# yh-jun/SNR-Aligned_diffSE

Measured on AMD Instinct MI355X. Metric: utterances/sec (4 s @16 kHz, N=30 PC steps) at 1/2/4/8 MI355X; PESQ delta vs ref, higher is better.
Workload: dtype fp16; 1 GPU; C2: B=32 4 s/16 kHz clips per GPU, N=30 PC steps (reverse_diffusion + ald, 60 NFE/utt), OUVE SDE, NCSN++ nf=128, fp16; global_batch=32, per_gpu_batch=32, seq_len=512, parallelism=dp1 (utterance sharding)

## Files before the change

### snr-aligned_diffse_amd/csrc/conv.hip

```cpp
#include "conv_common.h"

#include <algorithm>
#include <type_traits>

using namespace snrse_conv;

namespace {

template <int NWM, int BN>
SNRSE_DEV void block_stats_flush(const ConvParams& p, const float* red, int blk_b, int blk_n0) {
  asm volatile("s_waitcnt lgkmcnt(0)" ::: "memory");
  __builtin_amdgcn_s_barrier();
  const int slot = blockIdx.x & (SNRSE_STAT_SLOTS - 1);
  for (int t = threadIdx.x; t < 2 * BN; t += blockDim.x) {
    float a = 0.f;
#pragma unroll
    for (int w = 0; w < NWM; ++w) a += red[w * 2 * BN + t];
    if (blk_n0 + (t >> 1) < p.Cout)
      unsafeAtomicAdd(&p.stats[stat_idx(blk_b, slot, blk_n0 + (t >> 1), p.Cout) + (t & 1)], (double)a);
  }
}

template <typename TO, int NWM, int BN, bool DEFER = false, int LA = 8>
SNRSE_DEV void epilogue_lds(const ConvParams& p, const f32x4 (&acc)[4][4], int mb, int nb, int lane, float* stage,
// ... 21 lines not shown
    bias[k] = (p.bias && nok) ? p.bias[n + k] : 0.f;
    cb[k] = 0.f;
    cw[k][0] = cw[k][1] = cw[k][2] = cw[k][3] = 0.f;
    if (p.comb_src && nok) {
      cw[k][0] = p.comb_w[(n + k) * 4 + 0]; cw[k][1] = p.comb_w[(n + k) * 4 + 1];
      cw[k][2] = p.comb_w[(n + k) * 4 + 2]; cw[k][3] = p.comb_w[(n + k) * 4 + 3];
      cb[k] = p.comb_b[n + k];
    }
  }
  const int m_last = min(mb + nvalid - 1, p.M - 1);
  const bool one_b = mb < p.M && (mb / HW) == (m_last / HW);
  const int slot = blockIdx.x & (SNRSE_STAT_SLOTS - 1);
  const bool seg = p.stats && !one_b && HW % RPP == 0;
  int seg_b = -1;
  if (p.temb && one_b && nok) {
    const float* tb = p.temb + (size_t)(mb / HW) * p.temb_stride + n;
#pragma unroll
    for (int k = 0; k < EPC; ++k) bias[k] += tb[k];
  }
  constexpr int NPASS = 64 / RPP;
  static_assert(LA >= 1 && LA <= NPASS, "lookahead");
  u32x4 rpre[NPASS];
  f32x4 qpre[NPASS];
  auto epi_issue = [&](int pass) {
    const int row = r0 + pass * RPP;
    const int m = mb + row;
    if (m < p.M && nok && row < nvalid) {
      if (p.res) rpre[pass] = *(const u32x4*)((const TO*)p.res + (size_t)m * p.res_ld + n);
      if (p.comb_src) qpre[pass] = *(const f32x4*)(p.comb_src + (size_t)m * 4);
    }
  };
#pragma unroll
  for (int pass = 0; pass < LA; ++pass) epi_issue(pass);
  float s1[EPC], s2[EPC];
#pragma unroll
  for (int k = 0; k < EPC; ++k) { s1[k] = 0.f; s2[k] = 0.f; }
  auto seg_flush = [&]() {
#pragma unroll
    for (int k = 0; k < EPC; ++k) {
#pragma unroll
      for (int o = NCH; o < 64; o <<= 1) {
        s1[k] += __shfl_xor(s1[k], o, 64);
        s2[k] += __shfl_xor(s2[k], o, 64);
      }
    }
    if (r0 == 0 && nok && seg_b >= 0 && (long long)seg_b * HW < p.M) {
      const size_t base = stat_idx(seg_b, slot, n, p.Cout);
#pragma unroll
      for (int k = 0; k < EPC; ++k) {
        unsafeAtomicAdd(&p.stats[base + 2 * k], (double)s1[k]);
        unsafeAtomicAdd(&p.stats[base + 2 * k + 1], (double)s2[k]);
      }
    }
#pragma unroll
    for (int k = 0; k < EPC; ++k) { s1[k] = 0.f; s2[k] = 0.f; }
  };
#pragma unroll
  for (int pass = 0; pass < NPASS; ++pass) {
    if (pass + LA < NPASS) epi_issue(pass + LA);
    const int row = r0 + pass * RPP;
    const int m = mb + row;
    if (seg) {
      const int bp = (mb + pass * RPP) / HW;
      if (bp != seg_b) {
        if (seg_b >= 0) seg_flush();
        seg_b = bp;
      }
    }
    if (m >= p.M || !nok || row >= nvalid) continue;
    float v[EPC];
    const float* sr = stage + row * LDR + cc * EPC;
#pragma unroll
    for (int k = 0; k < EPC; ++k) v[k] = sr[k] + bias[k];
    if (p.temb && !one_b) {
      const float* tb = p.temb + (size_t)(m / HW) * p.temb_stride + n;
#pragma unroll
      for (int k = 0; k < EPC; ++k) v[k] += tb[k];
    }
    if (p.res) epi_residual<TO>(rpre[pass], v);
#pragma unroll
    for (int k = 0; k < EPC; ++k) v[k] *= p.out_scale;
    if (p.comb_src) {
      const f32x4 q = qpre[pass];
#pragma unroll
      for (int k = 0; k < EPC; ++k) v[k] += q[0] * cw[k][0] + q[1] * cw[k][1] + q[2] * cw[k][2] + q[3] * cw[k][3] + cb[k];
    }
    const u32x4 o = epi_pack<TO>(v);
    if (p.epi_nt)
      __builtin_nontemporal_store(o, (u32x4*)((TO*)p.out + (size_t)m * p.out_ld + n));
    else
      *(u32x4*)((TO*)p.out + (size_t)m * p.out_ld + n) = o;
    if (p.stats) {
      if (one_b || seg) {
#pragma unroll
        for (int k = 0; k < EPC; ++k) { s1[k] += v[k]; s2[k] = fmaf(v[k], v[k], s2[k]); }
      } else {
#pragma unroll
        for (int k = 0; k < EPC; ++k) {
          const size_t o = stat_idx(m / HW, slot, n + k, p.Cout);
          unsafeAtomicAdd(&p.stats[o], (double)v[k]);
          unsafeAtomicAdd(&p.stats[o + 1], (double)v[k] * v[k]);
        }
      }
    }
  }
  if (seg && seg_b >= 0) seg_flush();
  if (p.stats && one_b) {
#pragma unroll
    for (int k = 0; k < EPC; ++k) {
#pragma unroll
      for (int o = NCH; o < 64; o <<= 1) {
        s1[k] += __shfl_xor(s1[k], o, 64);
        s2[k] += __shfl_xor(s2[k], o, 64);
      }
    }
  }
  if (p.stats && blk_b >= 0) {
    if (r0 == 0) {
#pragma unroll
      for (int k = 0; k < EPC; ++k) {
        red[(wm * BN + nb - blk_n0 + cc * EPC + k) * 2] = s1[k];
        red[(wm * BN + nb - blk_n0 + cc * EPC + k) * 2 + 1] = s2[k];
      }
    }
    if constexpr (!DEFER) block_stats_flush<NWM, BN>(p, red, blk_b, blk_n0);
  } else if (p.stats && one_b && r0 == 0 && nok) {
    const size_t base = stat_idx(mb / HW, slot, n, p.Cout);
#pragma unroll
    for (int k = 0; k < EPC; ++k) {
      unsafeAtomicAdd(&p.stats[base + 2 * k], (double)s1[k]);
      unsafeAtomicAdd(&p.stats[base + 2 * k + 1], (double)s2[k]);
    }
  }
}

template <int S>
SNRSE_DEV float sum_lanes_strided(float v) {
  static_assert(S == 8 || S == 16, "lane stride");
  if constexpr (S == 8)
    v += __int_as_float(__builtin_amdgcn_update_dpp(0, __float_as_int(v), 0x128, 0xf, 0xf, false));
  const auto r = __builtin_amdgcn_permlane16_swap(__float_as_uint(v), __float_as_uint(v), false, false);
  v = __uint_as_float(r[0]) + __uint_as_float(r[1]);
  const auto r2 = __builtin_amdgcn_permlane32_swap(__float_as_uint(v), __float_as_uint(v), false, false);
  return __uint_as_float(r2[0]) + __uint_as_float(r2[1]);
}


template <int TW>
SNRSE_DEV int epi_pix(int mb, int row, int seg_skip) {
  return TW == 64 ? mb + row : mb + row + (row / TW) * seg_skip;
}

template <typename TO, int EF>
SNRSE_DEV void epi_add(const ConvParams& p, int nb, int lane, int b, float (&add)[16 / sizeof(TO)]) {
  constexpr int EPC = 16 / (int)sizeof(TO);
  const int n = nb + (lane % (64 / EPC)) * EPC;
  const bool f_temb = EF < 0 ? p.temb != nullptr : (EF & EF_TEMB) != 0;
#pragma unroll
  for (int k = 0; k < EPC; ++k) add[k] = 0.f;
  if (p.bias) {
#pragma unroll
    for (int k = 0; k < EPC; k += 4) {
      const f32x4 v = *(const f32x4*)(p.bias + n + k);
      add[k] = v[0]; add[k + 1] = v[1]; add[k + 2] = v[2]; add[k + 3] = v[3];
    }
  }
  if (f_temb) {
    const float* tb = p.temb + (size_t)b * p.temb_stride + n;
#pragma unroll
    for (int k = 0; k < EPC; ++k) add[k] += tb[k];
  }
}

template <typename TO, int NWM, int BN, bool DEFER, int EF = EF_RT, int TW = 64, int LA = 8>
SNRSE_DEV void epilogue_img(const ConvParams& p, const f32x4 (&acc)[4][4], int mb, int nb, int lane, float* stage,
                            float* red, int wm, int b, int blk_n0, int seg_skip = 0,
                            const float* pre_add = nullptr) {
  const bool f_res = EF < 0 ? p.res != nullptr : (EF & EF_RES) != 0;
  const bool f_comb = EF < 0 ? p.comb_src != nullptr : (EF & EF_COMB) != 0;
  const bool f_stats = EF < 0 ? p.stats != nullptr : (EF & EF_STATS) != 0;
  const bool f_nt = EF < 0 ? p.epi_nt != 0 : (EF & EF_NT) != 0;
  constexpr int LDR = 68;
  constexpr int EPC = 16 / (int)sizeof(TO);
  constexpr int NCH = 64 / EPC;
  constexpr int RPP = 64 / NCH;
  const int lrow = lane & 15, lg = lane >> 4;
#pragma unroll
  for (int i = 0; i < 4; ++i)
#pragma unroll
    for (int j = 0; j < 4; ++j)
#pragma unroll
      for (int e = 0; e < 4; ++e) stage[(i * 16 + lg * 4 + e) * LDR + j * 16 + lrow] = acc[i][j][e];
  const int cc = lane % NCH, r0 = lane / NCH;
  const int n = nb + cc * EPC;
  float add[EPC];
  if (pre_add) {
#pragma unroll
    for (int k = 0; k < EPC; ++k) add[k] = pre_add[k];
  } else {
    epi_add<TO, EF>(p, nb, lane, b, add);
  }
  float cw[EPC][4], cb[EPC];
  if (f_comb) {
#pragma unroll
    for (int k = 0; k < EPC; ++k) {
      const f32x4 w = *(const f32x4*)(p.comb_w + (size_t)(n + k) * 4);
      cw[k][0] = w[0]; cw[k][1] = w[1]; cw[k][2] = w[2]; cw[k][3] = w[3];
      cb[k] = p.comb_b[n + k];
    }
  }
  float s1[EPC], s2[EPC];
#pragma unroll
  for (int k = 0; k < EPC; ++k) { s1[k] = 0.f; s2[k] = 0.f; }
  constexpr int NPASS = 64 / RPP;
  static_assert(LA >= 1 && LA <= NPASS, "lookahead");
  u32x4 rpre[NPASS];
  f32x4 qpre[NPASS];
  auto epi_issue = [&](int pass) {
    const size_t m = (size_t)epi_pix<TW>(mb, r0 + pass * RPP, seg_skip);
    if (f_res) rpre[pass] = *(const u32x4*)((const TO*)p.res + m * p.res_ld + n);
    if (f_comb) qpre[pass] = *(const f32x4*)(p.comb_src + m * 4);
  };
#pragma unroll
  for (int pass = 0; pass < LA; ++pass) epi_issue(pass);
  __builtin_amdgcn_s_waitcnt(0xc07f);
  __builtin_amdgcn_wave_barrier();
#pragma unroll
  for (int pass = 0; pass < NPASS; ++pass) {
    if (pass + LA < NPASS) epi_issue(pass + LA);
    const int row = r0 + pass * RPP;
    const size_t m = (size_t)epi_pix<TW>(mb, row, seg_skip);
    float v[EPC];
    const float* sr = stage + row * LDR + cc * EPC;
#pragma unroll
    for (int k = 0; k < EPC; ++k) v[k] = sr[k] + add[k];
    if (f_res) epi_residual<TO>(rpre[pass], v);
    if (p.out_scale != 1.f) {
#pragma unroll
      for (int k = 0; k < EPC; ++k) v[k] *= p.out_scale;
    }
    if (f_comb) {
      const f32x4 q = qpre[pass];
#pragma unroll
      for (int k = 0; k < EPC; ++k) v[k] += q[0] * cw[k][0] + q[1] * cw[k][1] + q[2] * cw[k][2] + q[3] * cw[k][3] + cb[k];
    }
    const u32x4 o = epi_pack<TO>(v);
    if (f_nt)
      __builtin_nontemporal_store(o, (u32x4*)((TO*)p.out + m * p.out_ld + n));
    else
      *(u32x4*)((TO*)p.out + m * p.out_ld + n) = o;
    if (f_stats) {
#pragma unroll
      for (int k = 0; k < EPC; ++k) { s1[k] += v[k]; s2[k] = fmaf(v[k], v[k], s2[k]); }
    }
  }
  if (f_stats) {
#pragma unroll
    for (int k = 0; k < EPC; ++k) {
      s1[k] = sum_lanes_strided<NCH>(s1[k]);
      s2[k] = sum_lanes_strided<NCH>(s2[k]);
    }
    if (r0 == 0) {
#pragma unroll
      for (int k = 0; k < EPC; ++k) {
        red[(wm * BN + nb - blk_n0 + cc * EPC + k) * 2] = s1[k];
        red[(wm * BN + nb - blk_n0 + cc * EPC + k) * 2 + 1] = s2[k];
      }
    }
    if constexpr (!DEFER) block_stats_flush<NWM, BN>(p, red, b, blk_n0);
  }
}

template <typename TO, int FM, int FN>
SNRSE_DEV void epilogue(const ConvParams& p, const f32x4 (&acc)[FM][FN], int mb, int nb, int lane) {
  const int lrow = lane & 15, lg = lane >> 4;
  const int HW = p.H * p.W;
  const int m_last = min(mb + FM * 16, p.M) - 1;
  const bool one_b = mb < p.M && (mb / HW) == (m_last / HW);
#pragma unroll
  for (int j = 0; j < FN; ++j) {
    const int n = nb + j * 16 + lrow;
    const bool nok = n < p.Cout;
    const float bn = (p.bias && nok) ? p.bias[n] : 0.f;
    float cw0 = 0.f, cw1 = 0.f, cw2 = 0.f, cw3 = 0.f, cb = 0.f;
    if (p.comb_src && nok) {
      cw0 = p.comb_w[n * 4 + 0]; cw1 = p.comb_w[n * 4 + 1];
      cw2 = p.comb_w[n * 4 + 2]; cw3 = p.comb_w[n * 4 + 3];
      cb = p.comb_b[n];
    }
    float s1 = 0.f, s2 = 0.f;
#pragma unroll
    for (int i = 0; i < FM; ++i) {
#pragma unroll
      for (int e = 0; e < 4; ++e) {
        const int m = mb + i * 16 + lg * 4 + e;
        if (m >= p.M || !nok) continue;
        float v = acc[i][j][e] + bn;
        if (p.temb) v += p.temb[(size_t)(m / HW) * p.temb_stride + n];
        if (p.res) v += Elem<TO>::to_f(((const TO*)p.res)[(size_t)m * p.res_ld + n]);
        v *= p.out_scale;
        if (p.comb_src) {
          const float* q = p.comb_src + (size_t)m * 4;
          v += q[0] * cw0 + q[1] * cw1 + q[2] * cw2 + q[3] * cw3 + cb;
        }
        ((TO*)p.out)[(size_t)m * p.out_ld + n] = Elem<TO>::from_f(v);
        if (p.stats) {
          if (one_b) {
            s1 += v;
            s2 = fmaf(v, v, s2);
          } else {
            const size_t o = stat_idx(m / HW, blockIdx.x & (SNRSE_STAT_SLOTS - 1), n, p.Cout);
            unsafeAtomicAdd(&p.stats[o], (double)v);
            unsafeAtomicAdd(&p.stats[o + 1], (double)v * v);
          }
        }
      }
    }
    if (p.stats && one_b) {
      s1 += __shfl_xor(s1, 16, 64);
      s1 += __shfl_xor(s1, 32, 64);
      s2 += __shfl_xor(s2, 16, 64);
      s2 += __shfl_xor(s2, 32, 64);
      if (lg == 0 && nok) {
// ... 733 lines not shown
    const char* sb = sa + A_BYTES;
#pragma unroll
    for (int s = 0; s < 2; ++s) {
      u32x4 af[FM], bfr[FN];
#pragma unroll
      for (int i = 0; i < FM; ++i) af[i] = *(const u32x4*)(sa + swz(wm * TM + i * 16 + lrow, 4 * s + lg));
#pragma unroll
      for (int j = 0; j < FN; ++j) bfr[j] = *(const u32x4*)(sb + swz(wn * TN + j * 16 + lrow, 4 * s + lg));
#pragma unroll
      for (int i = 0; i < FM; ++i)
#pragma unroll
        for (int j = 0; j < FN; ++j) acc[i][j] = mfma_chunk<T>(af[i], bfr[j], acc[i][j]);
    }
    stage = stage == STAGES - 1 ? 0 : stage + 1;
  }
#undef SNRSE_ISSUE
  if (p.ksplit > 1) {
    float* const wsp = p.ws + (size_t)ks * p.M * p.Cout;
#pragma unroll
    for (int i = 0; i < FM; ++i)
#pragma unroll
      for (int e = 0; e < 4; ++e) {
        const int m = m0 + wm * TM + i * 16 + lg * 4 + e;
        if (m < p.M) {
#pragma unroll
          for (int j = 0; j < FN; ++j) wsp[(size_t)m * p.Cout + n0 + wn * TN + j * 16 + lrow] = acc[i][j][e];
        }
      }
    return;
  }
  asm volatile("s_waitcnt vmcnt(0) lgkmcnt(0)" ::: "memory");
  __builtin_amdgcn_s_barrier();
  const int b_lo = m0 / HW, b_hi = (min(m0 + BM, p.M) - 1) / HW;
  epilogue_lds<TO, WM, BN, false, sizeof(TO) == 2 ? 8 : 1>(p, acc, m0 + wm * TM, n0 + wn * TN, lane, (float*)(smem + wid * (64 * 68 * 4)),
                           (float*)(smem + 8 * (64 * 68 * 4)), wm, b_lo == b_hi ? b_lo : -1, n0);
}

template <typename TO>
__global__ __launch_bounds__(256) void conv_splitk_finalize(ConvParams p, int ppb) {
  __shared__ float red[16 * 256];
  const int HW = p.H * p.W;
  const int nbi = (HW + ppb - 1) / ppb;
  const int b = blockIdx.x / nbi;
  const int px0 = (blockIdx.x - b * nbi) * ppb, px1 = min(HW, px0 + ppb);
  const int cl = (threadIdx.x & 15) * 8, r0 = threadIdx.x >> 4;
  const int n = blockIdx.y * 128 + cl;
  float add[8], cw[8][4], cb[8], s1[8], s2[8];
#pragma unroll
  for (int k = 0; k < 8; ++k) {
    add[k] = (p.bias ? p.bias[n + k] : 0.f) + (p.temb ? p.temb[(size_t)b * p.temb_stride + n + k] : 0.f);
    s1[k] = 0.f;
    s2[k] = 0.f;
    cb[k] = 0.f;
    cw[k][0] = cw[k][1] = cw[k][2] = cw[k][3] = 0.f;
    if (p.comb_src) {
      cw[k][0] = p.comb_w[(n + k) * 4 + 0];
      cw[k][1] = p.comb_w[(n + k) * 4 + 1];
      cw[k][2] = p.comb_w[(n + k) * 4 + 2];
      cw[k][3] = p.comb_w[(n + k) * 4 + 3];
      cb[k] = p.comb_b[n + k];
    }
  }
  const size_t plane = (size_t)p.M * p.Cout;
  for (int px = px0 + r0; px < px1; px += 16) {
    const size_t m = (size_t)b * HW + px;
    const float* w = p.ws + m * p.Cout + n;
    f32x4 a0 = *(const f32x4*)w, a1 = *(const f32x4*)(w + 4);
    int s = 1;
    for (; s + 4 <= p.ksplit; s += 4) {
      f32x4 q[4][2];
#pragma unroll
      for (int u = 0; u < 4; ++u) {
        q[u][0] = *(const f32x4*)(w + (s + u) * plane);
        q[u][1] = *(const f32x4*)(w + (s + u) * plane + 4);
      }
#pragma unroll
      for (int u = 0; u < 4; ++u) {
        a0 += q[u][0];
        a1 += q[u][1];
      }
    }
    for (; s < p.ksplit; ++s) {
      a0 += *(const f32x4*)(w + s * plane);
      a1 += *(const f32x4*)(w + s * plane + 4);
    }
    float v[8];
#pragma unroll
    for (int k = 0; k < 4; ++k) {
      v[k] = a0[k] + add[k];
      v[4 + k] = a1[k] + add[4 + k];
    }
    if (p.res) {
      if constexpr (sizeof(TO) == 2) {
        epi_residual<TO>(*(const u32x4*)((const TO*)p.res + m * p.res_ld + n), v);
      } else {
        const float* rp = (const float*)p.res + m * p.res_ld + n;
#pragma unroll
        for (int k = 0; k < 8; ++k) v[k] += rp[k];
      }
    }
#pragma unroll
    for (int k = 0; k < 8; ++k) v[k] *= p.out_scale;
    if (p.comb_src) {
      const f32x4 q = *(const f32x4*)(p.comb_src + m * 4);
#pragma unroll
      for (int k = 0; k < 8; ++k) v[k] += q[0] * cw[k][0] + q[1] * cw[k][1] + q[2] * cw[k][2] + q[3] * cw[k][3] + cb[k];
    }
    if constexpr (sizeof(TO) == 2) {
      *(u32x4*)((TO*)p.out + m * p.out_ld + n) = epi_pack<TO>(v);
    } else {
      float* op = (float*)p.out + m * p.out_ld + n;
#pragma unroll
      for (int k = 0; k < 8; ++k) op[k] = v[k];
    }
#pragma unroll
    for (int k = 0; k < 8; ++k) {
      s1[k] += v[k];
      s2[k] = fmaf(v[k], v[k], s2[k]);
    }
  }
  if (p.stats) {
#pragma unroll
    for (int k = 0; k < 8; ++k) {
      red[r0 * 256 + (cl + k) * 2] = s1[k];
      red[r0 * 256 + (cl + k) * 2 + 1] = s2[k];
    }
    __syncthreads();
    const int t = threadIdx.x;
    float a = 0.f;
#pragma unroll
    for (int r = 0; r < 16; ++r) a += red[r * 256 + t];
    unsafeAtomicAdd(&p.stats[stat_idx(b, blockIdx.x & (SNRSE_STAT_SLOTS - 1), blockIdx.y * 128 + (t >> 1), p.Cout) +
                             (t & 1)],
                    (double)a);
  }
}


template <typename T, typename TO, int GNM, int EF, int TW, bool SCD>
__global__ __launch_bounds__(256, 2) void conv_halo5_kernel(ConvParams p) {
  constexpr int TH = 256 / TW, HC = TW + 2;
  constexpr int RW = TH / 4;
  constexpr int HROWS = (TH + 2) * HC;
  constexpr int HJ = (HROWS + 63) / 64;
  constexpr int HALO_BYTES = HROWS * 64;
  constexpr int TAPB = 128 * 64;
  constexpr int SLOT = 3 * TAPB;
  constexpr int KT = 32;
  static_assert(64 * HJ >= HROWS, "halo rows");
  extern __shared__ __attribute__((aligned(16))) char smem[];
  char* const halo = smem;
  char* const ring = smem + HALO_BYTES;
  float* const gnl = (float*)(smem + HALO_BYTES + 2 * SLOT + 1024);

  const int tid = threadIdx.x, lane = tid & 63;
  const int wid = __builtin_amdgcn_readfirstlane(tid >> 6);
#ifdef SNRSE_STAMPS
  constexpr int kStampOff = (HALO_BYTES + 2 * SLOT + 1280) > (4 * (64 * 68 * 4) + 4 * 128 * 2 * 4)
                                ? (HALO_BYTES + 2 * SLOT + 1280) : (4 * (64 * 68 * 4) + 4 * 128 * 2 * 4);
  unsigned long long* const lst = (unsigned long long*)(smem + kStampOff) + wid * 32;
#endif
  SNRSE_STAMP(0);
  const int wg = xcd_block_id(blockIdx.x, gridDim.x);
  const int n0 = (wg % p.ntn) * 128;
  int tile = wg / p.ntn;
  const int ntw = p.W / TW, nth = p.H / TH;
  const int w0 = (tile % ntw) * TW;
  tile /= ntw;
  const int h0 = (tile % nth) * TH;
  const int bb = tile / nth;

  const int Cin = p.C0 + p.C1;
  const int cbm = Cin / KT;
  const int Csc_all = p.Csc + p.Csc1;
  const int cbs = p.sc_src ? Csc_all / KT : 0;
  const int nq = 3 * cbm + cbs;
  const int K1 = 9 * Cin;
  const int hcol = tid & 3;

  const int rl = lane >> 2, swz8 = ((lane & 3) ^ ((rl >> 1) & 3)) * 8;
  const __amdgpu_buffer_rsrc_t wrsrc = make_rsrc(p.wgt, p.wbytes);
  const unsigned wlane = (unsigned)(((n0 + wid * 16 + rl) * K1 + swz8) * 2);
  const unsigned wrow64 = (unsigned)(64 * K1 * 2), wtap = (unsigned)(Cin * 2);
  using lds_ptr = __attribute__((address_space(3))) void*;
  auto dma_w = [&](auto k_, unsigned vl, unsigned soff, char* dst) {
    constexpr int k = decltype(k_)::value;
    __builtin_amdgcn_raw_ptr_buffer_load_lds(wrsrc, (lds_ptr)(dst + (k >> 1) * TAPB + (wid + 4 * (k & 1)) * 1024), 16,
                                             vl, soff + (k & 1) * wrow64 + (k >> 1) * wtap, 0, 0);
  };
  auto woff = [&](int c, int g) { return (unsigned)((3 * g * Cin + c * KT) * 2); };

  u32x4 hv[HJ];
  f32x4 gnv;
  auto gn_load = [&](int c) {
    if constexpr (GNM > 0) {
      if (tid < 16)
        gnv = *(const f32x4*)((tid < 8 ? p.gn_scale : p.gn_shift) + (size_t)bb * Cin + c * KT + (tid & 7) * 4);
    }
  };

  static_for<6>([&](auto k) { dma_w(k, wlane, 0u, ring); });
  gn_load(0);
  __builtin_amdgcn_sched_barrier(0);

  int hpix[HJ];
  bool hok[HJ];
#pragma unroll
  for (int j = 0; j < HJ; ++j) {
    const int hr = (tid >> 2) + 64 * j;
    const int hy = hr / HC, hx = hr - (hr / HC) * HC;
    const int ih = h0 + hy - 1, iw = w0 + hx - 1;
    hok[j] = hr < HROWS && ih >= 0 && ih < p.H && iw >= 0 && iw < p.W;
    hpix[j] = (bb * p.H + ih) * p.W + iw;
  }

#define SNRSE_HALO5_LOADS(BASE_, BYTES_, CS_, CC_)                                                     \
  do {                                                                                              \
    const __amdgpu_buffer_rsrc_t r_ = make_rsrc((BASE_), (BYTES_));                                 \
    const int cs_ = (CS_), cc_ = (CC_) + hcol * 8;                                                  \
    _Pragma("unroll") for (int j = 0; j < HJ; ++j) {                                                \
      const int voff_ = hok[j] ? (hpix[j] * cs_ + cc_) * 2 : (int)0x80000000;                       \
      hv[j] = __builtin_amdgcn_raw_buffer_load_b128(r_, voff_, 0, 0);                               \
    }                                                                                               \
  } while (0)
  auto halo_load = [&](int c) {
    const int ch = c * KT;
    const bool s1 = ch >= p.C0;
    SNRSE_HALO5_LOADS(s1 ? p.src1 : p.src0, s1 ? p.bytes1 : p.bytes0, s1 ? p.C1 : p.C0, s1 ? ch - p.C0 : ch);
  };
#undef SNRSE_HALO5_LOADS
  auto gn_publish = [&]() {
    if constexpr (GNM > 0) {
      if (tid < 16) {
        f32x4 g = gnv;
        if constexpr (GNM == 2) g *= kNegLog2e;
        *(f32x4*)(gnl + tid * 4) = g;
      }
    }
  };
  auto halo_store = [&](int c) {
    const bool tr = GNM > 0;
    float gsc[8], gsh[8];
    if constexpr (GNM > 0) {
      if (tr) {
        const f32x4 s0 = *(const f32x4*)(gnl + hcol * 8), s1 = *(const f32x4*)(gnl + hcol * 8 + 4);
        const f32x4 t0 = *(const f32x4*)(gnl + 32 + hcol * 8), t1 = *(const f32x4*)(gnl + 32 + hcol * 8 + 4);
#pragma unroll
        for (int i = 0; i < 4; ++i) { gsc[i] = s0[i]; gsc[4 + i] = s1[i]; gsh[i] = t0[i]; gsh[4 + i] = t1[i]; }
      }
    }
#pragma unroll
    for (int j = 0; j < HJ; ++j) {
      const int hr = (tid >> 2) + 64 * j;
      if (j == HJ - 1 && hr >= HROWS) break;
      u32x4 v = hv[j];
      if constexpr (GNM > 0) {
        if (tr) v = gn_xform8<T, GNM>(v, gsc, gsh, hok[j]);
      }
      *(u32x4*)(halo + swz64(hr, hcol)) = v;
    }
  };
  f32x4 acc[2][4][4];
#pragma unroll
  for (int h = 0; h < 2; ++h)
#pragma unroll
    for (int i = 0; i < 4; ++i)
#pragma unroll
      for (int j = 0; j < 4; ++j) acc[h][i][j] = f32x4{0.f, 0.f, 0.f, 0.f};
  const int lrow = lane & 15, lg = lane >> 4;
  auto vm_after_dma = [&]() { __builtin_amdgcn_s_waitcnt(0x0f76); };


  if constexpr (SCD) {
    const int kq = cbs / cbm, kr = cbs - kq * cbm;
    int krem = 0;
    auto nsc_next = [&]() {
      krem += kr;
      const bool wrap = krem >= cbm;
      if (wrap) krem -= cbm;
      return kq + (wrap ? 1 : 0);
    };
    auto kind_of = [](int s, int k, int& su) -> int {
      su = 0;
      if (k >= 3) {
        if (s == 0 || s == 2 || s == 4) return s >> 1;
        su = s <= 3 ? s >> 1 : s - 3;
        return 3;
      }
      if (s < 2) return s;
      if (k == 0) return 2;
      if (k == 1) {
        if (s == 2) return 2;
        return 3;
      }
      if (s == 3) return 2;
      su = s == 2 ? 0 : 1;
      return 3;
    };
    auto m2_pos = [](int k) { return k >= 3 ? 4 : k == 2 ? 3 : 2; };
    const __amdgpu_buffer_rsrc_t scrsrc = make_rsrc(p.sc_wgt, p.sc_wbytes);
    const __amdgpu_buffer_rsrc_t xrsrc0 = make_rsrc(p.sc_src, p.sc_bytes0), xrsrc1 = make_rsrc(p.sc_src1, p.sc_bytes1);
    const unsigned sclane = (unsigned)(((n0 + wid * 16 + rl) * Csc_all + swz8) * 2);
    const unsigned scrow64 = (unsigned)(64 * Csc_all * 2);
    const int trow = wid * 16 + rl;
    const int xpix = (bb * p.H + h0 + trow / TW) * p.W + w0 + trow % TW;
    halo_load(0);
    if constexpr (GNM > 0) {
      gn_publish();
      __syncthreads();
    }
    halo_store(0);
    const bool w0g = GNM > 0 && wid == 0;
    bool halo_inflight = false;
    int c = 0, pos = 0, k = nsc_next(), ub = 0;
    int su, kind = kind_of(0, k, su);
    for (int q = 0; q < nq; ++q) {
      int c2 = c, pos2 = pos + 1, k2 = k, ub2 = ub;
      if (pos2 == 3 + k) { c2 = c + 1; pos2 = 0; ub2 = ub + k; k2 = c2 < cbm ? nsc_next() : 0; }
      int su2;
      const int kind2 = kind_of(pos2, k2, su2);
      if (halo_inflight) {
        if (w0g) asm volatile("s_waitcnt vmcnt(%0) lgkmcnt(0)" ::"n"(HJ + 1) : "memory");
        else asm volatile("s_waitcnt vmcnt(%0) lgkmcnt(0)" ::"n"(HJ) : "memory");
      } else {
        asm volatile("s_waitcnt vmcnt(0) lgkmcnt(0)" ::: "memory");
      }
      __builtin_amdgcn_s_barrier();
      char* const nx = ring + ((q + 1) & 1) * SLOT;
      __amdgpu_buffer_rsrc_t Rc, Rn;
      unsigned Vc, Vn, Sc, Sn, Oc, On, DPn;
      int DDn;
      char* Dc = nx + wid * 1024;
      char* Dn = Dc + TAPB;
      if (kind2 < 3) {
        const bool fin = q + 1 >= nq;
        Rc = Rn = wrsrc;
        Vc = Vn = fin ? wlane | 0x80000000u : wlane;
        Sc = fin ? 0u : woff(c2, kind2);
        Sn = Sc + wtap; DPn = wtap; DDn = TAPB;
        Oc = On = wrow64;
      } else {
        const int kb = (ub2 + su2) * KT;
        const bool one = kb >= p.Csc;
        const int cs = one ? p.Csc1 : p.Csc, cb = one ? kb - p.Csc : kb;
        const unsigned xstep = (unsigned)((64 / TW) * p.W * cs * 2);
        Rc = scrsrc; Vc = sclane; Sc = (unsigned)(kb * 2); Oc = scrow64;
        Rn = one ? xrsrc1 : xrsrc0;
        Vn = (unsigned)((xpix * cs + swz8) * 2);
        Sn = (unsigned)(cb * 2); On = xstep; DPn = 2 * xstep; DDn = 8192;
      }
      auto dma_pair = [&]() {
        __builtin_amdgcn_raw_ptr_buffer_load_lds(Rc, (lds_ptr)Dc, 16, Vc, Sc, 0, 0);
        __builtin_amdgcn_raw_ptr_buffer_load_lds(Rc, (lds_ptr)(Dc + 4096), 16, Vc, Sc + Oc, 0, 0);
        Rc = Rn; Vc = Vn; Sc = Sn; Oc = On; Dc = Dn;
        Sn += DPn; Dn += DDn;
      };
      const char* sl = ring + (q & 1) * SLOT;
      const bool mainph = kind < 3;
      const char* abuf = mainph ? halo : sl + TAPB;
      const int ntap = mainph ? 3 : 1, rs = mainph ? HC : TW;
      const int arow0 = mainph ? (wid * RW + kind) * HC + lrow : wid * RW * TW + lrow;
      auto tap_body = [&](int jt, auto gap_) {
        constexpr bool gap = decltype(gap_)::value;
        const int arow = arow0 + jt;
        const char* sb = sl + jt * TAPB;
        u32x4 af[4], bfr[8];
#pragma unroll
        for (int i = 0; i < 4; ++i) af[i] = *(const u32x4*)(abuf + swz64(arow + (16 * i / TW) * rs + (16 * i) % TW, lg));
#pragma unroll
        for (int j = 0; j < 8; ++j) bfr[j] = *(const u32x4*)(sb + swz64(j * 16 + lrow, lg));
        static_for<32>([&](auto m_) {
          constexpr int m = decltype(m_)::value, h = m >> 4, i = (m >> 2) & 3, j = m & 3;
          acc[h][i][j] = mfma_chunk<T>(af[i], bfr[h * 4 + j], acc[h][i][j]);
          if constexpr (gap && (m & 7) == 7 && m < 24) dma_pair();
        });
        if constexpr (gap) {
#pragma unroll
          for (int u = 0; u < 3; ++u) {
            __builtin_amdgcn_sched_group_barrier(0x008, 8, 0);
            __builtin_amdgcn_sched_group_barrier(0x020, 2, 0);
          }
          __builtin_amdgcn_sched_group_barrier(0x008, 8, 0);
        }
      };
      tap_body(0, std::true_type{});
#pragma nounroll
      for (int jt = 1; jt < ntap; ++jt) tap_body(jt, std::false_type{});
      if (kind == 0 && c + 1 < cbm) {
        vm_after_dma();
        halo_load(c + 1);
        gn_load(c + 1);
        halo_inflight = true;
      } else {
        halo_inflight = false;
      }
      if (c + 1 < cbm) {
        if (kind == 2) {
          gn_publish();
          if (k == 0) {
            asm volatile("s_waitcnt lgkmcnt(0)" ::: "memory");
            __builtin_amdgcn_s_barrier();
            vm_after_dma();
            halo_store(c + 1);
          }
        } else if (kind == 3 && pos == m2_pos(k) + 1) {
          vm_after_dma();
          halo_store(c + 1);
        }
      }
      c = c2; pos = pos2; k = k2; ub = ub2; kind = kind2; su = su2;
    }
  } else {
  halo_load(0);
  if constexpr (GNM > 0) {
    gn_publish();
    __syncthreads();
  }
  halo_store(0);
  SNRSE_STAMP(1);
  bool halo_inflight = false;
  const bool w0g = GNM > 0 && wid == 0;
  int c = 0, g = 0;
  unsigned soff = woff(0, 1);
  const unsigned soff_g = 3 * wtap, soff_c = (unsigned)(2 * KT) - 6 * wtap;
  for (int q = 0; q < nq; ++q) {
    const bool first = g == 0, last = g == 2;
    if (halo_inflight) {
      if (w0g) asm volatile("s_waitcnt vmcnt(%0) lgkmcnt(0)" ::"n"(HJ + 1) : "memory");
      else asm volatile("s_waitcnt vmcnt(%0) lgkmcnt(0)" ::"n"(HJ) : "memory");
    } else {
      asm volatile("s_waitcnt vmcnt(0) lgkmcnt(0)" ::: "memory");
    }
    __builtin_amdgcn_s_barrier();
    SNRSE_STAMP(2 + 2 * (q & 15));
    const bool fin = q + 1 >= nq;
    const unsigned vl = fin ? wlane | 0x80000000u : wlane, so = fin ? 0u : soff;
    char* const nx = ring + ((q + 1) & 1) * SLOT;
    const char* sl = ring + (q & 1) * SLOT;
    const int hrow = (wid * RW + g) * HC + lrow;
    static_for<3>([&](auto jt_) {
      constexpr int jt = decltype(jt_)::value;
      const int hbase = hrow + jt;
      const char* sb = sl + jt * TAPB;
      u32x4 af[4], bfr[8];
#pragma unroll
      for (int i = 0; i < 4; ++i) af[i] = *(const u32x4*)(halo + swz64(hbase + (16 * i / TW) * HC + (16 * i) % TW, lg));
#pragma unroll
      for (int j = 0; j < 8; ++j) bfr[j] = *(const u32x4*)(sb + swz64(j * 16 + lrow, lg));
      static_for<32>([&](auto m_) {
        constexpr int m = decltype(m_)::value, h = m >> 4, i = (m >> 2) & 3, j = m & 3;
        acc[h][i][j] = mfma_chunk<T>(af[i], bfr[h * 4 + j], acc[h][i][j]);
        if constexpr (jt < 2 && (m & 7) == 7 && m < 24)
          dma_w(std::integral_constant<int, 3 * jt + (m >> 3)>{}, vl, so, nx);
      });
    });
    static_assert(sizeof(T) == 2, "one MFMA per mfma_chunk");
#pragma unroll
    for (int t = 0; t < 2; ++t) {
#pragma unroll
      for (int u = 0; u < 3; ++u) {
        __builtin_amdgcn_sched_group_barrier(0x008, 8, 0);
        __builtin_amdgcn_sched_group_barrier(0x020, 1, 0);
      }
      __builtin_amdgcn_sched_group_barrier(0x008, 8, 0);
    }
    __builtin_amdgcn_sched_group_barrier(0x008, 32, 0);
    SNRSE_STAMP(3 + 2 * (q & 15));
    if (first && c + 1 < cbm) {
      vm_after_dma();
      halo_load(c + 1);
      gn_load(c + 1);
      halo_inflight = true;
    } else {
      halo_inflight = false;
    }
    if (last && c + 1 < cbm) {
      gn_publish();
      asm volatile("s_waitcnt lgkmcnt(0)" ::: "memory");
      __builtin_amdgcn_s_barrier();
      vm_after_dma();
      halo_store(c + 1);
    }
    soff += g == 1 ? soff_c : soff_g;
    if (last) { g = 0; ++c; }
    else ++g;
  }
  }
  SNRSE_STAMP(28);
  float add0[16 / sizeof(TO)], add1[16 / sizeof(TO)];
  epi_add<TO, EF>(p, n0, lane, bb, add0);
  epi_add<TO, EF>(p, n0 + 64, lane, bb, add1);
  asm volatile("s_waitcnt vmcnt(0) lgkmcnt(0)" ::: "memory");
  __builtin_amdgcn_s_barrier();
  float* const stage = (float*)(smem + wid * (64 * 68 * 4));
  float* const red = (float*)(smem + 4 * (64 * 68 * 4));
  const int mrow = (bb * p.H + h0 + wid * RW) * p.W + w0;
  constexpr int ELA = sizeof(TO) == 2 ? 8 : 2;
  epilogue_img<TO, 4, 128, true, EF, TW, ELA>(p, acc[0], mrow, n0, lane, stage, red, wid, bb, n0, p.W - TW, add0);
  asm volatile("s_waitcnt lgkmcnt(0)" ::: "memory");
  __builtin_amdgcn_wave_barrier();
  SNRSE_STAMP(26);
  epilogue_img<TO, 4, 128, true, EF, TW, ELA>(p, acc[1], mrow, n0 + 64, lane, stage, red, wid, bb, n0, p.W - TW, add1);
  SNRSE_STAMP(27);
  if (EF < 0 ? p.stats != nullptr : (EF & EF_STATS) != 0) block_stats_flush<4, 128>(p, red, bb, n0);
#ifdef SNRSE_STAMPS
  {
    unsigned long long st_[29];
    if (lane == 0)
      for (int i = 0; i < 29; ++i) st_[i] = lst[i];
    unsigned long long t_end;
    asm volatile("s_waitcnt vmcnt(0)\n\ts_memtime %0\n\ts_waitcnt lgkmcnt(0)" : "=s"(t_end)::"memory");
    unsigned hw, xcc;
    asm volatile("s_getreg_b32 %0, hwreg(HW_REG_HW_ID)" : "=s"(hw));
    asm volatile("s_getreg_b32 %0, hwreg(HW_REG_XCC_ID)" : "=s"(xcc));
    if (lane == 0 && p.stamps) {
      unsigned long long* g = p.stamps + ((size_t)blockIdx.x * 8 + wid) * 32;
      for (int i = 0; i < 29; ++i) g[i] = st_[i];
      g[29] = t_end;
      g[30] = hw;
      g[31] = xcc;
    }
  }
#endif
}


template <auto K, typename... Args>
int launch_dyn_lds(dim3 grid, dim3 block, size_t lds, hipStream_t s, const Args&... args) {
  static const hipError_t attr = hipFuncSetAttribute((const void*)K, hipFuncAttributeMaxDynamicSharedMemorySize, (int)lds);
  SNRSE_RET(attr);
  hipLaunchKernelGGL(K, grid, block, lds, s, args...);
  return (int)hipGetLastError();
}

template <typename TO>
int launch_splitk_finalize(const ConvParams& p, hipStream_t s) {
  const int HW = p.H * p.W, ppb = 64;
  hipLaunchKernelGGL((conv_splitk_finalize<TO>), dim3(p.B * ((HW + ppb - 1) / ppb), p.Cout / 128), dim3(256), 0, s, p,
                     ppb);
  return (int)hipGetLastError();
}

inline int k_tiles(const ConvParams& p, int KT) {
  return p.ksize * p.ksize * ((p.C0 + p.C1) / KT) + (p.sc_src ? (p.Csc + p.Csc1) / KT : 0);
}

inline int stream_output(const snrse_ctx& cx, long long bytes) {
  return cx.epi_nt == 2 ? bytes > ((long long)cx.epi_nt_mb << 20) : cx.epi_nt;
}

template <typename T, typename TO, int GNM, int EF, int TW, bool SCD>
int launch_halo5_ef(ConvParams p, int grid, hipStream_t s) {
  constexpr size_t main_lds = (256 / TW + 2) * (TW + 2) * 64 + 2 * 3 * 128 * 64 + 1024 + 256;
  constexpr size_t epi_lds = 4 * (64 * 68 * 4) + 4 * 128 * 2 * 4;
#ifdef SNRSE_STAMPS
  constexpr size_t lds = (main_lds > epi_lds ? main_lds : epi_lds) + 1024;
#else
  constexpr size_t lds = main_lds > epi_lds ? main_lds : epi_lds;
#endif
  return launch_dyn_lds<conv_halo5_kernel<T, TO, GNM, EF, TW, SCD>>(dim3(grid), dim3(256), lds, s, p);
}

template <typename T, typename TO, int GNM, int TW>
int launch_halo5_gn(ConvParams p, hipStream_t s, snrse_ctx& cx) {
  p.ntn = p.Cout / 128;
  p.epi_nt = stream_output(cx, (long long)p.M * p.out_ld * (long long)sizeof(TO));
  cx.last_epi_nt = p.epi_nt;
  const int tiles = p.B * (p.H / (256 / TW)) * (p.W / TW) * p.ntn;
  const int grid = tiles;
  const bool scd = p.sc_src != nullptr;
  if constexpr (sizeof(TO) == 2 && GNM != 1) {
    if (cx.h5_specialise && p.bias) {
#define SNRSE_H5_EF(F) \
  case (F): return launch_halo5_ef<T, TO, GNM, (F), TW, false>(p, grid, s);
#define SNRSE_H5_EFS(F) \
  case (F): return launch_halo5_ef<T, TO, GNM, (F), TW, true>(p, grid, s);
      if (!scd) {
        switch (epi_flags(p)) {
          SNRSE_H5_EF(EF_TEMB | EF_STATS)
          SNRSE_H5_EF(EF_TEMB | EF_STATS | EF_NT)
          SNRSE_H5_EF(EF_RES | EF_STATS)
          SNRSE_H5_EF(EF_RES | EF_STATS | EF_NT)
          SNRSE_H5_EF(EF_STATS)
          SNRSE_H5_EF(EF_STATS | EF_NT)
          SNRSE_H5_EF(EF_TEMB)
          default: break;
        }
      } else {
        switch (epi_flags(p)) {
          SNRSE_H5_EFS(EF_STATS)
          SNRSE_H5_EFS(EF_STATS | EF_NT)
          SNRSE_H5_EFS(EF_COMB | EF_STATS)
          default: break;
        }
      }
#undef SNRSE_H5_EF
#undef SNRSE_H5_EFS
    }
  }
  return scd ? launch_halo5_ef<T, TO, GNM, EF_RT, TW, true>(p, grid, s)
             : launch_halo5_ef<T, TO, GNM, EF_RT, TW, false>(p, grid, s);
}

template <typename T, typename TO, int TW>
int launch_halo5_tw(ConvParams p, hipStream_t s, snrse_ctx& cx) {
  cx.last_tw = TW;
  if (!p.gn_scale) return launch_halo5_gn<T, TO, 0, TW>(p, s, cx);
  if (!p.gn_act) return launch_halo5_gn<T, TO, 1, TW>(p, s, cx);
  return launch_halo5_gn<T, TO, 2, TW>(p, s, cx);
}

inline bool halo_tile32(const ConvParams& p) { return p.H % 8 == 0 && p.W % 32 == 0; }
inline bool halo_tile64(const ConvParams& p) { return p.H % 4 == 0 && p.W % 64 == 0; }

template <typename T, typename TO>
int launch_halo5(ConvParams p, hipStream_t s, snrse_ctx& cx) {
  if (halo_tile32(p) && cx.h5_tw != 64) return launch_halo5_tw<T, TO, 32>(p, s, cx);
  return launch_halo5_tw<T, TO, 64>(p, s, cx);
}

int choose_ksplit(const ConvParams& p, int tiles, int nk, const snrse_ctx& cx, int min_kt = 4) {
  if (!cx.splitk || !cx.ws || tiles >= cx.splitk_target * 3 / 4) return 1;
  int s = (cx.splitk_target + tiles - 1) / tiles;
  if (s > nk / min_kt) s = nk / min_kt;
  const size_t plane = (size_t)p.M * p.Cout * sizeof(float);
  if ((size_t)s * plane > cx.ws_bytes) s = (int)(cx.ws_bytes / plane);
  return s >= 2 ? s : 1;
}

template <typename T, typename TO, int BM, int BN, int WM, int WN>
int launch_conv(ConvParams p, int npad, hipStream_t s, snrse_ctx& cx) {
  p.ntn = npad / BN;
  const int tiles = ((p.M + BM - 1) / BM) * p.ntn;
  p.ksplit = (sizeof(T) == 4 && BN == 128 && p.Cout % 128 == 0)
                 ? choose_ksplit(p, tiles, k_tiles(p, ConvTraits<T>::KT), cx, 2) : 1;
  p.ws = cx.ws;
  cx.last_ksplit = p.ksplit;
  const size_t lds = (size_t)2 * (BM + BN) * 128;
  hipLaunchKernelGGL((conv_mfma_kernel<T, TO, BM, BN, WM, WN>), dim3(tiles * p.ksplit), dim3(64 * WM * WN), lds, s, p);
  if (p.ksplit == 1) return (int)hipGetLastError();
  SNRSE_LAUNCH_CHECK();
  return launch_splitk_finalize<TO>(p, s);
}

template <int BM, int BN, int WM, int WN>
int launch_x3(ConvParams p, hipStream_t s, snrse_ctx& cx) {
  constexpr size_t main_lds = (size_t)2 * (BM + BN) * 128;
  constexpr size_t epi_lds = (BM / WM == 64 && BN / WN == 64) ? (size_t)WM * WN * 64 * 68 * 4 + WM * BN * 2 * 4 : 0;
  constexpr size_t lds = main_lds > epi_lds ? main_lds : epi_lds;
  p.ntn = (p.Cout + BN - 1) / BN;
  const int tiles = ((p.M + BM - 1) / BM) * p.ntn;
  p.ksplit = BN == 128 ? choose_ksplit(p, tiles, k_tiles(p, SplitBf16Opnd::KT), cx, 2) : 1;
  p.ws = cx.ws;
  cx.last_ksplit = p.ksplit;
  const int rc = launch_dyn_lds<conv_x3_kernel<BM, BN, WM, WN>>(dim3(tiles * p.ksplit), dim3(64 * WM * WN), lds, s, p);
  if (rc || p.ksplit == 1) return rc;
  return launch_splitk_finalize<float>(p, s);
}

template <int GNM, int SPR, int TWV, int EF = EF_RT>
int launch_x3h_ef(ConvParams p, hipStream_t s, int tiles) {
  p.ntn = p.Cout / 128;
  p.ksplit = 1;
  return launch_dyn_lds<conv_x3h_kernel<GNM, SPR, TWV, EF>>(dim3(tiles), dim3(512), X3G<TWV, SPR>::LDS, s, p);
}

template <int GNM, int SPR, int TWV>
int launch_x3h_gn(const ConvParams& p, hipStream_t s, int tiles, bool spec) {
  if constexpr (GNM != 1 && SPR == 2 && TWV == 32) {
    if (spec && p.bias) {
      switch (epi_flags(p)) {
        case EF_TEMB | EF_STATS: return launch_x3h_ef<GNM, SPR, TWV, EF_TEMB | EF_STATS>(p, s, tiles);
        case EF_TEMB | EF_STATS | EF_NT: return launch_x3h_ef<GNM, SPR, TWV, EF_TEMB | EF_STATS | EF_NT>(p, s, tiles);
        case EF_RES | EF_STATS: return launch_x3h_ef<GNM, SPR, TWV, EF_RES | EF_STATS>(p, s, tiles);
        case EF_RES | EF_STATS | EF_NT: return launch_x3h_ef<GNM, SPR, TWV, EF_RES | EF_STATS | EF_NT>(p, s, tiles);
        case EF_STATS: return launch_x3h_ef<GNM, SPR, TWV, EF_STATS>(p, s, tiles);
        case EF_STATS | EF_NT: return launch_x3h_ef<GNM, SPR, TWV, EF_STATS | EF_NT>(p, s, tiles);
        case EF_COMB | EF_STATS: return launch_x3h_ef<GNM, SPR, TWV, EF_COMB | EF_STATS>(p, s, tiles);
        case EF_COMB | EF_STATS | EF_NT: return launch_x3h_ef<GNM, SPR, TWV, EF_COMB | EF_STATS | EF_NT>(p, s, tiles);
        default: break;
      }
    }
  }
  return launch_x3h_ef<GNM, SPR, TWV>(p, s, tiles);
}

template <int SPR, int TWV>
int launch_x3h_spr(const ConvParams& p, hipStream_t s, int tiles, bool spec) {
  if (!p.gn_scale) return launch_x3h_gn<0, SPR, TWV>(p, s, tiles, spec);
  if (!p.gn_act) return launch_x3h_gn<1, SPR, TWV>(p, s, tiles, spec);
  return launch_x3h_gn<2, SPR, TWV>(p, s, tiles, spec);
}

int launch_x3h(const ConvParams& p, hipStream_t s, int tiles, int spread, int tw, bool spec) {
  if (spread == 2 && !(tw == 32 && ((p.C0 + p.C1) / 32) % 2 == 0)) spread = 1;
  if (tw == 32) {
    if (spread == 2) return launch_x3h_spr<2, 32>(p, s, tiles, spec);
    return spread ? launch_x3h_spr<1, 32>(p, s, tiles, spec) : launch_x3h_spr<0, 32>(p, s, tiles, spec);
  }
  return spread ? launch_x3h_spr<1, 64>(p, s, tiles, spec) : launch_x3h_spr<0, 64>(p, s, tiles, spec);
}

template <int BM, int BN, typename T, typename TO>
int launch_glds(ConvParams p, hipStream_t s, snrse_ctx& cx) {
  constexpr size_t lds = (size_t)3 * (BM + BN) * 128;
  p.ntn = p.Cout / BN;
  const int ntm = (p.M + BM - 1) / BM;
  p.ksplit = choose_ksplit(p, ntm * p.ntn, k_tiles(p, 64), cx);
  p.ws = cx.ws;
  cx.last_ksplit = p.ksplit;
  const int rc = launch_dyn_lds<conv_glds_kernel<BM, BN, T, TO>>(dim3(ntm * p.ntn * p.ksplit), dim3(512), lds, s, p);
  if (rc || p.ksplit == 1) return rc;
// ... 193 lines not shown
```

Baseline: 14.34 utt/s.

## Write fp16 halo5 conv epilogue directly from registers, skipping LDS staging

```diff
diff --git a/snr-aligned_diffse_amd/csrc/conv.hip b/snr-aligned_diffse_amd/csrc/conv.hip
--- a/snr-aligned_diffse_amd/csrc/conv.hip
+++ b/snr-aligned_diffse_amd/csrc/conv.hip
@@ -197,9 +197,8 @@
 }
 
 template <typename TO, int EF>
-SNRSE_DEV void epi_add(const ConvParams& p, int nb, int lane, int b, float (&add)[16 / sizeof(TO)]) {
+SNRSE_DEV void epi_add_n(const ConvParams& p, int n, int b, float (&add)[16 / sizeof(TO)]) {
   constexpr int EPC = 16 / (int)sizeof(TO);
-  const int n = nb + (lane % (64 / EPC)) * EPC;
   const bool f_temb = EF < 0 ? p.temb != nullptr : (EF & EF_TEMB) != 0;
 #pragma unroll
   for (int k = 0; k < EPC; ++k) add[k] = 0.f;
@@ -214,6 +213,90 @@
     const float* tb = p.temb + (size_t)b * p.temb_stride + n;
 #pragma unroll
     for (int k = 0; k < EPC; ++k) add[k] += tb[k];
+  }
+}
+template <typename TO, int EF>
+SNRSE_DEV void epi_add(const ConvParams& p, int nb, int lane, int b, float (&add)[16 / sizeof(TO)]) {
+  constexpr int EPC = 16 / (int)sizeof(TO);
+  epi_add_n<TO, EF>(p, nb + (lane % (64 / EPC)) * EPC, b, add);
+}
+
+template <typename TO, int EF, int TW>
+SNRSE_DEV void epilogue_reg(const ConvParams& p, const f32x4 (&acc)[2][4][4], int mb, int n0, int lane, float* red,
+                            int b, int seg_skip) {
+  static_assert(sizeof(TO) == 2, "8 couts per 16-B vector");
+  const bool f_res = EF < 0 ? p.res != nullptr : (EF & EF_RES) != 0;
+  const bool f_comb = EF < 0 ? p.comb_src != nullptr : (EF & EF_COMB) != 0;
+  const bool f_stats = EF < 0 ? p.stats != nullptr : (EF & EF_STATS) != 0;
+  const bool f_nt = EF < 0 ? p.epi_nt != 0 : (EF & EF_NT) != 0;
+  const int lrow = lane & 15, lg = lane >> 4;
+  const int n = n0 + 8 * lrow;
+  float add[8];
+  epi_add_n<TO, EF>(p, n, b, add);
+  float cw[8][4], cb[8];
+  if (f_comb) {
+#pragma unroll
+    for (int k = 0; k < 8; ++k) {
+      const f32x4 w = *(const f32x4*)(p.comb_w + (size_t)(n + k) * 4);
+      cw[k][0] = w[0]; cw[k][1] = w[1]; cw[k][2] = w[2]; cw[k][3] = w[3];
+      cb[k] = p.comb_b[n + k];
+    }
+  }
+  constexpr int LA = (EF >= 0 && !(EF & EF_COMB)) ? 16 : 4;
+  constexpr int NPRE = EF < 0 ? 0 : ((EF & EF_RES) ? LA : 0) + ((EF & EF_COMB) ? LA : 0);
+  u32x4 rpre[16];
+  f32x4 qpre[16];
+  auto pix = [&](int t) { return (size_t)epi_pix<TW>(mb, 16 * (t >> 2) + 4 * lg + (t & 3), seg_skip); };
+  auto epi_issue = [&](int t) {
+    const size_t m = pix(t);
+    if (f_res) rpre[t] = *(const u32x4*)((const TO*)p.res + m * p.res_ld + n);
+    if (f_comb) qpre[t] = *(const f32x4*)(p.comb_src + m * 4);
+  };
+#pragma unroll
+  for (int t = 0; t < LA; ++t) epi_issue(t);
+  asm volatile("s_waitcnt vmcnt(%0)" ::"n"(NPRE) : "memory");
+  float s1[8], s2[8];
+#pragma unroll
+  for (int k = 0; k < 8; ++k) { s1[k] = 0.f; s2[k] = 0.f; }
+#pragma unroll
+  for (int t = 0; t < 16; ++t) {
+    if (t + LA < 16) epi_issue(t + LA);
+    const int i = t >> 2, e = t & 3;
+    const size_t m = pix(t);
+    float v[8];
+#pragma unroll
+    for (int k = 0; k < 8; ++k) v[k] = acc[k >> 2][i][k & 3][e] + add[k];
+    if (f_res) epi_residual<TO>(rpre[t], v);
+    if (p.out_scale != 1.f) {
+#pragma unroll
+      for (int k = 0; k < 8; ++k) v[k] *= p.out_scale;
+    }
+    if (f_comb) {
+      const f32x4 q = qpre[t];
+#pragma unroll
+      for (int k = 0; k < 8; ++k) v[k] += q[0] * cw[k][0] + q[1] * cw[k][1] + q[2] * cw[k][2] + q[3] * cw[k][3] + cb[k];
+    }
+    const u32x4 o = epi_pack<TO>(v);
+    if (f_nt)
+      __builtin_nontemporal_store(o, (u32x4*)((TO*)p.out + m * p.out_ld + n));
+    else
+      *(u32x4*)((TO*)p.out + m * p.out_ld + n) = o;
+    if (f_stats) {
+#pragma unroll
+      for (int k = 0; k < 8; ++k) { s1[k] += v[k]; s2[k] = fmaf(v[k], v[k], s2[k]); }
+    }
+  }
+  if (f_stats) {
+#pragma unroll
+    for (int k = 0; k < 8; ++k) {
+      s1[k] = sum_lanes_strided<16>(s1[k]);
+      s2[k] = sum_lanes_strided<16>(s2[k]);
+    }
+    if (lg == 0) {
+#pragma unroll
+      for (int k = 0; k < 8; k += 2)
+        *(f32x4*)(red + (8 * lrow + k) * 2) = f32x4{s1[k], s2[k], s1[k + 1], s2[k + 1]};
+    }
   }
 }
 
@@ -1253,12 +1336,15 @@
   char* const halo = smem;
   char* const ring = smem + HALO_BYTES;
   float* const gnl = (float*)(smem + HALO_BYTES + 2 * SLOT + 1024);
+  constexpr bool REGEPI = sizeof(TO) == 2;
+  constexpr int MAIN_BYTES = HALO_BYTES + 2 * SLOT + 1280;
+  constexpr int STAGE_BYTES = 4 * (64 * 68 * 4);
 
   const int tid = threadIdx.x, lane = tid & 63;
   const int wid = __builtin_amdgcn_readfirstlane(tid >> 6);
 #ifdef SNRSE_STAMPS
-  constexpr int kStampOff = (HALO_BYTES + 2 * SLOT + 1280) > (4 * (64 * 68 * 4) + 4 * 128 * 2 * 4)
-                                ? (HALO_BYTES + 2 * SLOT + 1280) : (4 * (64 * 68 * 4) + 4 * 128 * 2 * 4);
+  constexpr int kStampOff = REGEPI ? MAIN_BYTES + 4096
+                                   : (MAIN_BYTES > STAGE_BYTES + 4096 ? MAIN_BYTES : STAGE_BYTES + 4096);
   unsigned long long* const lst = (unsigned long long*)(smem + kStampOff) + wid * 32;
 #endif
   SNRSE_STAMP(0);
@@ -1281,8 +1367,10 @@
 
   const int rl = lane >> 2, swz8 = ((lane & 3) ^ ((rl >> 1) & 3)) * 8;
   const __amdgpu_buffer_rsrc_t wrsrc = make_rsrc(p.wgt, p.wbytes);
-  const unsigned wlane = (unsigned)(((n0 + wid * 16 + rl) * K1 + swz8) * 2);
-  const unsigned wrow64 = (unsigned)(64 * K1 * 2), wtap = (unsigned)(Cin * 2);
+  const int wr0 = REGEPI ? 8 * rl + wid : wid * 16 + rl;
+  constexpr int WODD = REGEPI ? 4 : 64;
+  const unsigned wlane = (unsigned)(((n0 + wr0) * K1 + swz8) * 2);
+  const unsigned wrow64 = (unsigned)(WODD * K1 * 2), wtap = (unsigned)(Cin * 2);
   using lds_ptr = __attribute__((address_space(3))) void*;
   auto dma_w = [&](auto k_, unsigned vl, unsigned soff, char* dst) {
     constexpr int k = decltype(k_)::value;
@@ -1401,8 +1489,8 @@
     auto m2_pos = [](int k) { return k >= 3 ? 4 : k == 2 ? 3 : 2; };
     const __amdgpu_buffer_rsrc_t scrsrc = make_rsrc(p.sc_wgt, p.sc_wbytes);
     const __amdgpu_buffer_rsrc_t xrsrc0 = make_rsrc(p.sc_src, p.sc_bytes0), xrsrc1 = make_rsrc(p.sc_src1, p.sc_bytes1);
-    const unsigned sclane = (unsigned)(((n0 + wid * 16 + rl) * Csc_all + swz8) * 2);
-    const unsigned scrow64 = (unsigned)(64 * Csc_all * 2);
+    const unsigned sclane = (unsigned)(((n0 + wr0) * Csc_all + swz8) * 2);
+    const unsigned scrow64 = (unsigned)(WODD * Csc_all * 2);
     const int trow = wid * 16 + rl;
     const int xpix = (bb * p.H + h0 + trow / TW) * p.W + w0 + trow % TW;
     halo_load(0);
@@ -1588,22 +1676,35 @@
   }
   }
   SNRSE_STAMP(28);
-  float add0[16 / sizeof(TO)], add1[16 / sizeof(TO)];
-  epi_add<TO, EF>(p, n0, lane, bb, add0);
-  epi_add<TO, EF>(p, n0 + 64, lane, bb, add1);
-  asm volatile("s_waitcnt vmcnt(0) lgkmcnt(0)" ::: "memory");
-  __builtin_amdgcn_s_barrier();
-  float* const stage = (float*)(smem + wid * (64 * 68 * 4));
-  float* const red = (float*)(smem + 4 * (64 * 68 * 4));
+#ifdef SNRSE_H5_SKIP_EPI
+  if (p.M > 0) {
+    asm volatile("s_waitcnt vmcnt(0)" ::: "memory");
+    return;
+  }
+#endif
   const int mrow = (bb * p.H + h0 + wid * RW) * p.W + w0;
-  constexpr int ELA = sizeof(TO) == 2 ? 8 : 2;
-  epilogue_img<TO, 4, 128, true, EF, TW, ELA>(p, acc[0], mrow, n0, lane, stage, red, wid, bb, n0, p.W - TW, add0);
-  asm volatile("s_waitcnt lgkmcnt(0)" ::: "memory");
-  __builtin_amdgcn_wave_barrier();
-  SNRSE_STAMP(26);
-  epilogue_img<TO, 4, 128, true, EF, TW, ELA>(p, acc[1], mrow, n0 + 64, lane, stage, red, wid, bb, n0, p.W - TW, add1);
-  SNRSE_STAMP(27);
-  if (EF < 0 ? p.stats != nullptr : (EF & EF_STATS) != 0) block_stats_flush<4, 128>(p, red, bb, n0);
+  if constexpr (REGEPI) {
+    float* const red = (float*)(smem + MAIN_BYTES);
+    epilogue_reg<TO, EF, TW>(p, acc, mrow, n0, lane, red + wid * 256, bb, p.W - TW);
+    SNRSE_STAMP(26);
+    SNRSE_STAMP(27);
+    if (EF < 0 ? p.stats != nullptr : (EF & EF_STATS) != 0) block_stats_flush<4, 128>(p, red, bb, n0);
+  } else {
+    float add0[16 / sizeof(TO)], add1[16 / sizeof(TO)];
+    epi_add<TO, EF>(p, n0, lane, bb, add0);
+    epi_add<TO, EF>(p, n0 + 64, lane, bb, add1);
+    asm volatile("s_waitcnt vmcnt(0) lgkmcnt(0)" ::: "memory");
+    __builtin_amdgcn_s_barrier();
+    float* const stage = (float*)(smem + wid * (64 * 68 * 4));
+    float* const red = (float*)(smem + STAGE_BYTES);
+    epilogue_img<TO, 4, 128, true, EF, TW, 2>(p, acc[0], mrow, n0, lane, stage, red, wid, bb, n0, p.W - TW, add0);
+    asm volatile("s_waitcnt lgkmcnt(0)" ::: "memory");
+    __builtin_amdgcn_wave_barrier();
+    SNRSE_STAMP(26);
+    epilogue_img<TO, 4, 128, true, EF, TW, 2>(p, acc[1], mrow, n0 + 64, lane, stage, red, wid, bb, n0, p.W - TW, add1);
+    SNRSE_STAMP(27);
+    if (EF < 0 ? p.stats != nullptr : (EF & EF_STATS) != 0) block_stats_flush<4, 128>(p, red, bb, n0);
+  }
 #ifdef SNRSE_STAMPS
   {
     unsigned long long st_[29];
@@ -1654,11 +1755,13 @@
 int launch_halo5_ef(ConvParams p, int grid, hipStream_t s) {
   constexpr size_t main_lds = (256 / TW + 2) * (TW + 2) * 64 + 2 * 3 * 128 * 64 + 1024 + 256;
   constexpr size_t epi_lds = 4 * (64 * 68 * 4) + 4 * 128 * 2 * 4;
+  constexpr size_t used_lds = sizeof(TO) == 2 ? main_lds + 4 * 128 * 2 * 4 : (main_lds > epi_lds ? main_lds : epi_lds);
 #ifdef SNRSE_STAMPS
-  constexpr size_t lds = (main_lds > epi_lds ? main_lds : epi_lds) + 1024;
+  constexpr size_t lds = used_lds + 1024;
 #else
-  constexpr size_t lds = main_lds > epi_lds ? main_lds : epi_lds;
+  constexpr size_t lds = used_lds;
 #endif
+  static_assert(lds <= 80 * 1024, "two workgroups per CU");
   return launch_dyn_lds<conv_halo5_kernel<T, TO, GNM, EF, TW, SCD>>(dim3(grid), dim3(256), lds, s, p);
 }
 
```

Result: faster. 14.63 utt/s (median of 6 runs) (+2.0%).
